# iamwangyabin/hardnetNas

Measured on AMD Instinct MI355X. Metric: Mpatches/s (32×32→128-D) at 1/2/4/8 MI355X; HPatches FPR95 parity, higher is better.
Workload: dtype bf16x3; 1 GPU; Stock HardNet forward, 262144 synthetic 32x32 patches per GPU; model=hardnet, global_batch=262144, per_gpu_batch=262144, parallelism=dp1

## Files before the change

hardnetnas_amd/csrc/hn_hardnet.hip:

```cpp
#include "hn_common.h"
#include "hn_internal.h"

#include <algorithm>
#include <cstdlib>

template <bool NORM>
__global__ __launch_bounds__(256) void k_stem(const float* __restrict__ in, float* __restrict__ out,
                                              const float* __restrict__ w,
                                              const float* __restrict__ b,
                                              float eps) {
  __shared__ float tile[34 * 34];
  __shared__ float red[8];
  const int t = threadIdx.x;
  const size_t p = blockIdx.x;
  const float4 v = reinterpret_cast<const float4*>(in + p * 1024)[t];
  for (int i = t; i < 34 * 34; i += 256) tile[i] = 0.f;
  float mean = 0.f, sd = 1.f;
  if (NORM) {
    float s = wave_sum(v.x + v.y + v.z + v.w);
    if ((t & 63) == 0) red[t >> 6] = s;
    __syncthreads();
    mean = (red[0] + red[1] + red[2] + red[3]) * (1.f / 1024.f);
    const float d0 = v.x - mean, d1 = v.y - mean, d2 = v.z - mean, d3 = v.w - mean;
    float q = wave_sum(d0 * d0 + d1 * d1 + d2 * d2 + d3 * d3);
// ... 756 lines not shown
      w0l[j] = (__bf16)(v - (float)w0h[j]);
    }
#pragma unroll
    for (int i = 0; i < 16; ++i) b16[i] = stem_b[8 * (i >> 2) + 4 * h + (i & 3)];
  }
  auto stem_loads = [&](int s) {
    int p0, y0;
    tile_of(s, p0, y0);
    if (p0 == cur_patch) return;
    const float4* pp = reinterpret_cast<const float4*>(in + (size_t)p0 * 1024) + lane;
    pv[0] = pp[0]; pv[1] = pp[64]; pv[2] = pp[128]; pv[3] = pp[192];
  };
  auto stem_write = [&](int s, char* dst) {
    int p0, y0;
    tile_of(s, p0, y0);
    if (p0 != cur_patch) {
    cur_patch = p0;
    float mean = 0.f, sd = 1.f;
    if (eps >= 0.f) {
      float a = 0.f;
#pragma unroll
      for (int k = 0; k < 4; ++k) a += (pv[k].x + pv[k].y) + (pv[k].z + pv[k].w);
      mean = wave_sum(a) * (1.f / 1024.f);
      float q = 0.f;
#pragma unroll
      for (int k = 0; k < 4; ++k) {
        const float d0 = pv[k].x - mean, d1 = pv[k].y - mean, d2 = pv[k].z - mean,
                    d3 = pv[k].w - mean;
        q += (d0 * d0 + d1 * d1) + (d2 * d2 + d3 * d3);
      }
      sd = sqrtf(wave_sum(q) * (1.f / 1023.f)) + eps;
    }
    const float inv = 1.f / sd;
#define HN_PUT(K)                                                                          \
  {                                                                                        \
    const int q4 = 4 * (lane + 64 * K), y = q4 >> 5, x = q4 & 31;                          \
    float* d = pt + (y + 1) * 34 + x + 1;                                                  \
    d[0] = (pv[K].x - mean) * inv; d[1] = (pv[K].y - mean) * inv;                           \
    d[2] = (pv[K].z - mean) * inv; d[3] = (pv[K].w - mean) * inv;                           \
  }
    HN_PUT(0) HN_PUT(1) HN_PUT(2) HN_PUT(3)
#undef HN_PUT
    }
    constexpr int NPIX = C::RIN * C::NCOLS;
    constexpr int NT0 = (NPIX + 31) / 32;
#pragma unroll 1
    for (int t = pw_; t < NT0; t += C::NWP) {
      const int pix = t * 32 + r;
      const int wr = pix / C::NCOLS, wc = pix % C::NCOLS;
      const int y = y0 - 1 + wr, x = wc - 1;
      const bool inside = pix < NPIX && (unsigned)y < 32u && (unsigned)x < 32u;
      const int yc = inside ? y : 0, xc = inside ? x : 0;
      bf16x8 xh, xl;
#pragma unroll
      for (int j = 0; j < 8; ++j) {
        const int tap = 8 * h + j;
        const float v = tap < 9 ? pt[(yc + tap / 3) * 34 + xc + tap % 3] : 0.f;
        xh[j] = (__bf16)v;
        xl[j] = (__bf16)(v - (float)xh[j]);
      }
      const f32x16 c0 = mfma3(w0h, w0l, xh, xl, f32x16{});
      if (pix < NPIX) {
        char* o = dst + wr * C::RS + wc * 80 + 8 * h;
#pragma unroll
        for (int q = 0; q < 4; ++q) {
          bf16x4 oh, ol;
#pragma unroll
          for (int j = 0; j < 4; ++j) {
            const float v = inside ? fmaxf(c0[4 * q + j] + b16[4 * q + j], 0.f) : 0.f;
            oh[j] = (__bf16)v;
            ol[j] = (__bf16)(v - (float)oh[j]);
          }
          *reinterpret_cast<uint2*>(o + 16 * q) = __builtin_bit_cast(uint2, oh);
          *reinterpret_cast<uint2*>(o + C::PLANE + 16 * q) = __builtin_bit_cast(uint2, ol);
        }
      }
    }
  };

  if (producer) {
    if constexpr (STEM) {
      static_assert(CIN == 32 && HIN == 32 && S == 1 && NP == 1, "stem fusion is conv1-only");
      for (int i = lane; i < 34 * 34; i += 64) pt[i] = 0.f;
      stem_loads(0);
      stem_write(0, buf0);
    } else {
      produce_loads(0, pf);
      produce_write(buf0, pf);
      if (NS > 1) produce_loads(1, pf);
    }
  } else {
    for (int i = tid; i < COUT; i += C::NWC * 64) reinterpret_cast<float*>(smem + C::BIAS_OFF)[i] = bias[i];
  }
  __syncthreads();

  if (producer) {
    if constexpr ((ABL & 32) != 0) {
    } else if constexpr ((ABL & 8) != 0) {
#pragma unroll 1
      for (int s = 0; s < NS; ++s) __syncthreads();
    } else if constexpr (STEM) {
#pragma unroll 1
      for (int s = 0; s < NS; ++s) {
        if (s + 1 < NS) {
          stem_loads(s + 1);
          stem_write(s + 1, (s & 1) ? buf0 : buf1);
        }
        __syncthreads();
      }
    } else if constexpr (!C::DEEP) {
#pragma unroll 1
      for (int s = 0; s < NS; ++s) {
        if (s + 1 < NS) {
          produce_write((s & 1) ? buf0 : buf1, pf);
          if (s + 2 < NS) produce_loads(s + 2, pf);
        }
        __syncthreads();
        if constexpr (PST)
          if (s % C::NCC == C::NCC - 1) pstore(s, (s & 1) ? buf1 : buf0);
      }
    } else {
#pragma unroll 1
      for (int s = 0; s < NS; s += 2) {
        if (s + 2 < NS) produce_loads(s + 2, pf2);
        if (s + 1 < NS) produce_write(buf1, pf);
        __syncthreads();
        if constexpr (PST)
          if (s % C::NCC == C::NCC - 1) pstore(s, buf0);
        if (s + 1 >= NS) break;
        if (s + 3 < NS) produce_loads(s + 3, pf);
        if (s + 2 < NS) produce_write(buf0, pf2);
        __syncthreads();
        if constexpr (PST)
          if ((s + 1) % C::NCC == C::NCC - 1) pstore(s + 1, buf1);
      }
    }
    return;
  }

  const int wm = wave / WN, wn = wave % WN;
  const float* const sbias = reinterpret_cast<const float*>(smem + C::BIAS_OFF);
  int abase[C::MT], ylr[C::MT];
#pragma unroll
  for (int mt = 0; mt < C::MT; ++mt) {
    const int m = (wm * C::MT + mt) * 32 + r;
    const int np = m / (TR * C::WOUT), rem = m % (TR * C::WOUT);
    const int yl = rem / C::WOUT, xo = rem % C::WOUT;
    abase[mt] = np * C::PS + yl * S * C::RS + xo * PX + (PX == 80 ? h * 16 : 0);
    ylr[mt] = yl;
  }
  constexpr unsigned CHUNK_BYTES = 9 * 2 * C::NTOT * 2 * 64 * 16;
  const __amdgpu_buffer_rsrc_t wr_ = make_rsrc(wp, C::NCC * CHUNK_BYTES);
  const unsigned wvoff = (wn * C::NT * 2 * 64 + lane) * 16;
  f32x16 acc[C::MT][C::NT];
#pragma unroll
  for (int mt = 0; mt < C::MT; ++mt)
#pragma unroll
    for (int nt = 0; nt < C::NT; ++nt) acc[mt][nt] = f32x16{};

  constexpr int NKS = 18;
  auto load_b = [&](int cc, int ksx, uint4 (&dst)[C::NT][2]) {
#pragma unroll
    for (int nt = 0; nt < C::NT; ++nt) {
      const unsigned k = cc * CHUNK_BYTES +
                         (((ABL & 1) ? 0 : ksx) * C::NTOT + nt) * 2 * 64 * 16;
      dst[nt][0] = buf_load16(wr_, wvoff, k);
      dst[nt][1] = buf_load16(wr_, wvoff, k + 64 * 16);
    }
  };
  constexpr int WD = 3;
  static_assert(NKS % WD == 0, "the weight ring runs on across stages");
  uint4 bq[WD][C::NT][2];
#pragma unroll
  for (int k = 0; k + 1 < WD; ++k) load_b(0, k, bq[k]);
#pragma unroll 1
  for (int s = 0; s < NS; ++s) {
    const char* cur = (s & 1) ? buf1 : buf0;
    const int cc = s % C::NCC, ccn = (s + 1) % C::NCC;
    uint4 aq[2][C::MT][2];
    auto load_a = [&](int ksx, uint4 (&dst)[C::MT][2]) {
      const int tap = (ABL & 2) ? 0 : ksx >> 1, ks = (ABL & 2) ? 0 : ksx & 1;
      const int toff = (tap / 3) * C::RS + C::colofs(tap % 3) * PX + (PX == 80 ? ks * 32 : 0);
#pragma unroll
      for (int mt = 0; mt < C::MT; ++mt) {
        const int co = PX == 80 ? 0 : 16 * ((2 * ks + h) ^ ((ylr[mt] + (tap / 3) / S) & 3));
        dst[mt][0] = *reinterpret_cast<const uint4*>(cur + abase[mt] + toff + co);
        dst[mt][1] = *reinterpret_cast<const uint4*>(cur + C::PLANE + abase[mt] + toff + co);
      }
    };
    load_a(0, aq[0]);
#pragma unroll
    for (int ksx = 0; ksx < NKS; ++ksx) {
      if (ksx + WD - 1 < NKS)
        load_b(cc, ksx + WD - 1, bq[(ksx + WD - 1) % WD]);
      else
        load_b(ccn, ksx + WD - 1 - NKS, bq[(ksx + WD - 1) % WD]);
      if (ksx + 1 < NKS) load_a(ksx + 1, aq[(ksx + 1) & 1]);
      __builtin_amdgcn_sched_barrier(0);
      if constexpr (PST) {
        if (ksx == 0 && cc == 0 && s > 0) __builtin_amdgcn_s_barrier();
      }
#pragma unroll
      for (int mt = 0; mt < C::MT; ++mt) {
        const bf16x8 xh = as_bf16x8(aq[ksx & 1][mt][0]), xl = as_bf16x8(aq[ksx & 1][mt][1]);
#pragma unroll
        for (int nt = 0; nt < C::NT; ++nt) {
          if constexpr (ABL & 16)
            acc[mt][nt][0] += __builtin_bit_cast(float, aq[ksx & 1][mt][0].x ^ aq[ksx & 1][mt][1].y ^
                                                           bq[ksx % WD][nt][0].z ^ bq[ksx % WD][nt][1].w);
          else
            acc[mt][nt] = mfma3(as_bf16x8(bq[ksx % WD][nt][0]), as_bf16x8(bq[ksx % WD][nt][1]), xh,
                                xl, acc[mt][nt]);
        }
      }
      __builtin_amdgcn_sched_barrier(0);
    }
    if (PST && cc == C::NCC - 1) {
      __syncthreads();
      char* stg = const_cast<char*>(cur);
#pragma unroll
      for (int nt = 0; nt < C::NT; ++nt) {
        float4 bv[4];
#pragma unroll
        for (int q = 0; q < 4; ++q)
          bv[q] = *reinterpret_cast<const float4*>(sbias + (wn * C::NT + nt) * 32 + 8 * q + 4 * h);
#pragma unroll
        for (int mt = 0; mt < C::MT; ++mt) {
          char* o = stage_at(stg, (wm * C::MT + mt) * 32 + r) + ((wn * C::NT + nt) * 32 + 4 * h) * 4;
#pragma unroll
          for (int q = 0; q < 4; ++q) {
            float4 v;
            v.x = fmaxf(acc[mt][nt][4 * q + 0] + bv[q].x, relu_lo);
            v.y = fmaxf(acc[mt][nt][4 * q + 1] + bv[q].y, relu_lo);
            v.z = fmaxf(acc[mt][nt][4 * q + 2] + bv[q].z, relu_lo);
            v.w = fmaxf(acc[mt][nt][4 * q + 3] + bv[q].w, relu_lo);
            *reinterpret_cast<float4*>(o + 32 * q) = v;
          }
          acc[mt][nt] = f32x16{};
        }
      }
      __syncthreads();
      continue;
    }
    if (cc == C::NCC - 1) {
      int p0, y0;
      tile_of(s, p0, y0);
      float* obase = out + ((size_t)(p0 * C::HOUT + y0) * C::WOUT + wm * C::MT * 32 + r) * COUT +
                     wn * C::NT * 32 + 4 * h;
#pragma unroll
      for (int nt = 0; nt < C::NT; ++nt) {
        float4 bv[4];
#pragma unroll
        for (int q = 0; q < 4; ++q)
          bv[q] = *reinterpret_cast<const float4*>(sbias + (wn * C::NT + nt) * 32 + 8 * q + 4 * h);
#pragma unroll
        for (int mt = 0; mt < C::MT; ++mt) {
          const bool ok = NP == 1 || p0 + ((wm * C::MT + mt) * 32) / (TR * C::WOUT) < P;
          if (ok) {
#pragma unroll
            for (int q = 0; q < 4; ++q) {
              float4 v;
              v.x = fmaxf(acc[mt][nt][4 * q + 0] + bv[q].x, relu_lo);
              v.y = fmaxf(acc[mt][nt][4 * q + 1] + bv[q].y, relu_lo);
              v.z = fmaxf(acc[mt][nt][4 * q + 2] + bv[q].z, relu_lo);
              v.w = fmaxf(acc[mt][nt][4 * q + 3] + bv[q].w, relu_lo);
              if constexpr (CST) {
                float* scr = reinterpret_cast<float*>(smem + 2 * C::BUF) + wave * (C::SCR / 4);
                *reinterpret_cast<float4*>(scr + r * C::SROW + 8 * q + 4 * h) = v;
              } else if (!(ABL & 4) || v.x == 1234.5f) {
                *reinterpret_cast<float4*>(obase + (size_t)mt * 32 * COUT + nt * 32 + 8 * q) = v;
              }
            }
          }
          if (CST && ok) {
            __builtin_amdgcn_wave_barrier();
            asm volatile("" ::: "memory");
            const float* scr = reinterpret_cast<const float*>(smem + 2 * C::BUF) + wave * (C::SCR / 4);
            float* ob = out + ((size_t)(p0 * C::HOUT + y0) * C::WOUT + (wm * C::MT + mt) * 32) * COUT +
                        (wn * C::NT + nt) * 32;
#pragma unroll
            for (int k = 0; k < 4; ++k) {
              const int pl = 8 * k + (lane >> 3), c4 = lane & 7;
              *reinterpret_cast<float4*>(ob + (size_t)pl * COUT + 4 * c4) =
                  *reinterpret_cast<const float4*>(scr + pl * C::SROW + 4 * c4);
            }
            __builtin_amdgcn_wave_barrier();
            asm volatile("" ::: "memory");
          }
          acc[mt][nt] = f32x16{};
        }
      }
    }
    if constexpr (!(ABL & 32)) __syncthreads();
  }
  if constexpr (PST) __builtin_amdgcn_s_barrier();
}

template <int K>
__global__ __launch_bounds__(256) void k_head(const float* __restrict__ a, float* __restrict__ out,
                                              const uint4* __restrict__ wp,
                                              const float* __restrict__ bias, int P, float l2eps) {
  __shared__ float ssq[2][64];
  const int tid = threadIdx.x, lane = tid & 63, wave = tid >> 6;
  const int wm = wave >> 1, wn = wave & 1;
  const int r = lane & 31, h = lane >> 5;
  const int pbase = blockIdx.x * 64 + wm * 32;
  const int pa = min(pbase + r, P - 1);
  const float* arow = a + (size_t)pa * K + h * 8;
  f32x16 acc[2] = {f32x16{}, f32x16{}};
#pragma unroll 4
  for (int ks = 0; ks < K / 16; ++ks) {
    const float4 x0 = *reinterpret_cast<const float4*>(arow + ks * 16);
    const float4 x1 = *reinterpret_cast<const float4*>(arow + ks * 16 + 4);
    uint4 hi, lo;
    split8(x0, x1, hi, lo);
    const bf16x8 ah = as_bf16x8(hi), al = as_bf16x8(lo);
#pragma unroll
    for (int nt = 0; nt < 2; ++nt) {
      const int idx = ((ks * 4 + wn * 2 + nt) * 2) * 64 + lane;
      acc[nt] = mfma3(ah, al, as_bf16x8(wp[idx]), as_bf16x8(wp[idx + 64]), acc[nt]);
    }
  }
  float b0 = bias[wn * 64 + r], b1 = bias[wn * 64 + 32 + r];
  float part[16];
#pragma unroll
  for (int i = 0; i < 16; ++i) {
    acc[0][i] += b0;
    acc[1][i] += b1;
    part[i] = half_sum(acc[0][i] * acc[0][i] + acc[1][i] * acc[1][i]);
  }
  if (r == 0) {
#pragma unroll
    for (int i = 0; i < 16; ++i) ssq[wn][wm * 32 + (i & 3) + 8 * (i >> 2) + 4 * h] = part[i];
  }
  __syncthreads();
#pragma unroll
  for (int i = 0; i < 16; ++i) {
    const int row = (i & 3) + 8 * (i >> 2) + 4 * h;
    const int p = pbase + row;
    const float norm = sqrtf(ssq[0][wm * 32 + row] + ssq[1][wm * 32 + row] + l2eps);
    if (p < P) {
      out[(size_t)p * 128 + wn * 64 + r] = acc[0][i] / norm;
      out[(size_t)p * 128 + wn * 64 + 32 + r] = acc[1][i] / norm;
    }
  }
}

template <int K, bool F16>
__global__ __launch_bounds__(256) void k_head2(const float* __restrict__ a, float* __restrict__ out,
                                               const uint4* __restrict__ wp,
                                               const float* __restrict__ bias, int P, float l2eps) {
  constexpr int KC = 32, NCH = K / KC;
  constexpr int AROW = 80;
  constexpr int APLANE = 64 * AROW;
  constexpr int ABYTES = 2 * APLANE;
  constexpr int BBYTES = 2 * 4 * 2 * 64 * 16;
  constexpr int BUF = ABYTES + BBYTES;
  __shared__ __attribute__((aligned(16))) char smem[2 * BUF];
  __shared__ float ssq[2][64];
  const int tid = threadIdx.x, lane = tid & 63, wave = tid >> 6;
  const int wm = wave >> 1, wn = wave & 1;
  const int r = lane & 31, h = lane >> 5;
  const int pbase = blockIdx.x * 64;
  const int arow0 = tid >> 3, acol = (tid & 7) * 4;
  const int pa0 = min(pbase + arow0, P - 1), pa1 = min(pbase + arow0 + 32, P - 1);
  float4 ra0, ra1;
  uint4 rb0, rb1, rb2, rb3;
#define HN_LOAD_CHUNK(c)                                                                   \
  {                                                                                        \
    ra0 = *reinterpret_cast<const float4*>(a + (size_t)pa0 * K + (c) * KC + acol);         \
    ra1 = *reinterpret_cast<const float4*>(a + (size_t)pa1 * K + (c) * KC + acol);         \
    const uint4* wc_ = wp + (size_t)(c) * 1024 + tid;                                      \
    rb0 = wc_[0]; rb1 = wc_[256]; rb2 = wc_[512]; rb3 = wc_[768];                          \
  }
  auto put_row = [&](char* buf, int row, const float4 v) {
    uint2 hv, lv;
    if (F16) {
      typedef _Float16 f16x4 __attribute__((ext_vector_type(4)));
      f16x4 hi, lo;
      hi[0] = (_Float16)v.x; lo[0] = (_Float16)(v.x - (float)hi[0]);
      hi[1] = (_Float16)v.y; lo[1] = (_Float16)(v.y - (float)hi[1]);
      hi[2] = (_Float16)v.z; lo[2] = (_Float16)(v.z - (float)hi[2]);
      hi[3] = (_Float16)v.w; lo[3] = (_Float16)(v.w - (float)hi[3]);
      hv = __builtin_bit_cast(uint2, hi);
      lv = __builtin_bit_cast(uint2, lo);
    } else {
      bf16x4 hi, lo;
      hi[0] = (__bf16)v.x; lo[0] = (__bf16)(v.x - (float)hi[0]);
      hi[1] = (__bf16)v.y; lo[1] = (__bf16)(v.y - (float)hi[1]);
      hi[2] = (__bf16)v.z; lo[2] = (__bf16)(v.z - (float)hi[2]);
      hi[3] = (__bf16)v.w; lo[3] = (__bf16)(v.w - (float)hi[3]);
      hv = __builtin_bit_cast(uint2, hi);
      lv = __builtin_bit_cast(uint2, lo);
    }
    *reinterpret_cast<uint2*>(buf + row * AROW + acol * 2) = hv;
    *reinterpret_cast<uint2*>(buf + APLANE + row * AROW + acol * 2) = lv;
  };
#define HN_STORE_CHUNK(buf)                                                                \
  {                                                                                        \
    put_row(buf, arow0, ra0);                                                              \
    put_row(buf, arow0 + 32, ra1);                                                         \
    uint4* bd_ = reinterpret_cast<uint4*>(buf + ABYTES) + tid;                             \
    bd_[0] = rb0; bd_[256] = rb1; bd_[512] = rb2; bd_[768] = rb3;                          \
  }
  f32x16 acc[2] = {f32x16{}, f32x16{}};
  HN_LOAD_CHUNK(0)
  HN_STORE_CHUNK(smem)
  __syncthreads();
#pragma unroll 1
  for (int c = 0; c < NCH; ++c) {
    const char* cur = smem + (c & 1) * BUF;
    if (c + 1 < NCH) HN_LOAD_CHUNK(c + 1)
#pragma unroll
    for (int ks = 0; ks < 2; ++ks) {
      const int aoff = (wm * 32 + r) * AROW + ks * 32 + h * 16;
      const uint4 ah = *reinterpret_cast<const uint4*>(cur + aoff);
      const uint4 al = *reinterpret_cast<const uint4*>(cur + APLANE + aoff);
#pragma unroll
      for (int nt = 0; nt < 2; ++nt) {
        const int boff = ABYTES + (((ks * 4 + wn * 2 + nt) * 2) * 64 + lane) * 16;
        const uint4 bh = *reinterpret_cast<const uint4*>(cur + boff);
        const uint4 bl = *reinterpret_cast<const uint4*>(cur + boff + 64 * 16);
        if (F16)
          acc[nt] = mfma3_f16(as_f16x8(ah), as_f16x8(al), as_f16x8(bh), as_f16x8(bl), acc[nt]);
        else
          acc[nt] = mfma3(as_bf16x8(ah), as_bf16x8(al), as_bf16x8(bh), as_bf16x8(bl), acc[nt]);
      }
    }
    if (c + 1 < NCH) HN_STORE_CHUNK(smem + ((c + 1) & 1) * BUF)
    __syncthreads();
  }
#undef HN_LOAD_CHUNK
#undef HN_STORE_CHUNK
  const float b0 = bias[wn * 64 + r], b1 = bias[wn * 64 + 32 + r];
  float part[16];
#pragma unroll
  for (int i = 0; i < 16; ++i) {
    acc[0][i] += b0;
    acc[1][i] += b1;
    part[i] = half_sum(acc[0][i] * acc[0][i] + acc[1][i] * acc[1][i]);
  }
  if (r == 0) {
#pragma unroll
    for (int i = 0; i < 16; ++i) ssq[wn][wm * 32 + (i & 3) + 8 * (i >> 2) + 4 * h] = part[i];
  }
  __syncthreads();
// ... 612 lines not shown
```

hardnetnas_amd/csrc/hn_wino1.hip:

```cpp
#include "hn_common.h"
#include "hn_internal.h"

namespace {

template <int CIN, int COUT, int H, int NP, int WM, int WN, bool CST>
struct W1Cfg {
  static constexpr int TR = H;
  static constexpr int NTX = H / 2;
  static constexpr int BM = NP * TR * NTX;
  static constexpr int MT = BM / WM / 32, NT = COUT / WN / 32;
  static constexpr int NTOT = COUT / 32, NCC = CIN / 32;
  static constexpr int XROW = NTX * 64;
  static constexpr int RS = 4 * XROW;
  static constexpr int PS = TR * RS;
  static constexpr int ZROW = NP * PS;
  static constexpr int PLANE = ZROW + RS;
  static constexpr int BUF = 2 * PLANE;
  static constexpr int NWC = WM * WN, NWP = 4, NTHR = (NWC + NWP) * 64, PTHR = NWP * 64;
  static constexpr int UNITS = NP * TR * NTX * 4;
  static_assert(64 % (4 * NTX) == 0 && PTHR % (4 * NTX) == 0, "a row's units share one wave");
  static constexpr int UPT = (UNITS + PTHR - 1) / PTHR;
  static constexpr bool DEEP = UPT <= 2;
  static constexpr int SROW = 36;
  static constexpr int SCR_OFF = 2 * BUF;
  static constexpr int SCR = CST ? 32 * SROW * 4 : 0;
  static constexpr int BIAS_OFF = SCR_OFF + NWC * SCR;
  static constexpr int SMEM = BIAS_OFF + COUT * 4;
  static constexpr int NKS = 24;
  static constexpr unsigned CHUNK_BYTES = NKS * NTOT * 2 * 64 * 16;
  static_assert(SMEM <= 160 * 1024, "LDS");
  static_assert(MT >= 1 && NT >= 1 && MT * WM * 32 == BM && NT * WN * 32 == COUT, "tiling");
  static_assert((TR * NTX) % 32 == 0 && 32 % NTX == 0, "an M tile = 32 / NTX whole rows of one patch");
  static_assert(RS % 256 == 0, "image rows on 256-byte boundaries (the bank-conflict argument)");
};

template <int CIN, int COUT, int H, int NP, int WM, int WN, bool CST, int WD = 3, int ABL = 0>
__global__ __launch_bounds__((WM * WN + 4) * 64) void k_conv_w1(const float* __restrict__ in, float* __restrict__ out,
                                                                const uint4* __restrict__ wp,
                                                                const float* __restrict__ bias, int P) {
  using C = W1Cfg<CIN, COUT, H, NP, WM, WN, CST>;
  constexpr int TR = C::TR;
  extern __shared__ __attribute__((aligned(16))) char smem[];
  const int tid = threadIdx.x, lane = tid & 63;
  const int wave = __builtin_amdgcn_readfirstlane(tid >> 6);
  const bool producer = wave >= C::NWC;
  const int r = lane & 31, h = lane >> 5;
  const int nwg = gridDim.x, rb = xcd_remap(blockIdx.x, nwg);
  const int ntiles = (P + NP - 1) / NP;
  const int my_tiles = rb < ntiles ? (ntiles - 1 - rb) / nwg + 1 : 0;
  const int NS = my_tiles * C::NCC;
  if (NS == 0) return;
  char* const buf0 = smem;
  char* const buf1 = smem + C::BUF;
  auto tile_of = [&](int s) { return (rb + (s / C::NCC) * nwg) * NP; };

  const int ptid = tid - C::NWC * 64;
  float4 pf[C::UPT][6], pf2[C::UPT][6];
  constexpr unsigned PATCH_BYTES = (unsigned)H * H * CIN * 4, OOB = 0x80000000u;
  auto produce_loads = [&](int s, float4 (&d)[C::UPT][6]) {
    const bool live = s < NS;
    const int p0 = live ? tile_of(s) : 0;
    const int cc = s % C::NCC;
    const int nval = !live ? 0 : P - p0 < NP ? P - p0 : NP;
    const __amdgpu_buffer_rsrc_t rs = make_rsrc(in + (size_t)p0 * H * H * CIN, (unsigned)nval * PATCH_BYTES);
#pragma unroll
    for (int k = 0; k < C::UPT; ++k) {
      const int u = ptid + k * C::PTHR;
      const int g = u & 3, t = (u >> 2) % C::NTX, rest = (u >> 2) / C::NTX;
      const int y = rest % TR, np = rest / TR;
      const bool rowok = C::UNITS % C::PTHR == 0 || u < C::UNITS;
#pragma unroll
      for (int j = 0; j < 3; ++j) {
        const int x = 2 * t - 1 + j;
        const bool ok = rowok && (j < 2 || t == C::NTX - 1) && (unsigned)x < (unsigned)H;
        const unsigned vo = ok ? (unsigned)(((np * H + y) * H + x) * CIN + cc * 32 + g * 8) * 4u : OOB;
        d[k][2 * j] = __builtin_bit_cast(float4, buf_load16(rs, vo, 0));
        d[k][2 * j + 1] = __builtin_bit_cast(float4, buf_load16(rs, vo, 16));
      }
    }
  };
  auto shfl4 = [&](const float4& v) {
    return make_float4(__shfl_down(v.x, 4, 64), __shfl_down(v.y, 4, 64), __shfl_down(v.z, 4, 64),
                       __shfl_down(v.w, 4, 64));
  };
  auto produce_write = [&](char* dst, const float4 (&d)[C::UPT][6]) {
#pragma unroll
    for (int k = 0; k < C::UPT; ++k) {
      const int u = ptid + k * C::PTHR;
      const int g = u & 3, t = (u >> 2) % C::NTX, rest = (u >> 2) / C::NTX;
      const int y = rest % TR, np = rest / TR;
      const bool last = t == C::NTX - 1;
      const float4 z = make_float4(0.f, 0.f, 0.f, 0.f);
      float4 dd[4][2];
#pragma unroll
      for (int i = 0; i < 2; ++i) {
        const float4 n0 = shfl4(d[k][i]), n1 = shfl4(d[k][2 + i]);
        dd[0][i] = d[k][i];
        dd[1][i] = d[k][2 + i];
        dd[2][i] = last ? d[k][4 + i] : n0;
        dd[3][i] = last ? z : n1;
      }
      if (C::UNITS % C::PTHR == 0 || u < C::UNITS) {
        const int off = np * C::PS + y * C::RS + t * 64 + 16 * (g ^ ((y + 1) & 3));
#pragma unroll
        for (int xi = 0; xi < 4; ++xi) {
          float4 v[2];
#pragma unroll
          for (int i = 0; i < 2; ++i) {
            const float4 d0 = dd[0][i], d1 = dd[1][i], d2 = dd[2][i], d3 = dd[3][i];
            if (xi == 0) v[i] = make_float4(d0.x - d2.x, d0.y - d2.y, d0.z - d2.z, d0.w - d2.w);
            if (xi == 1) v[i] = make_float4(d1.x + d2.x, d1.y + d2.y, d1.z + d2.z, d1.w + d2.w);
            if (xi == 2) v[i] = make_float4(d2.x - d1.x, d2.y - d1.y, d2.z - d1.z, d2.w - d1.w);
            if (xi == 3) v[i] = make_float4(d1.x - d3.x, d1.y - d3.y, d1.z - d3.z, d1.w - d3.w);
          }
          uint4 hi, lo;
          split8(v[0], v[1], hi, lo);
          *reinterpret_cast<uint4*>(dst + off + xi * C::XROW) = hi;
          *reinterpret_cast<uint4*>(dst + C::PLANE + off + xi * C::XROW) = lo;
        }
      }
    }
  };

  for (int i = tid; i < 4 * C::RS / 16; i += C::NTHR) {
    const int q = i / (C::RS / 16), o = (i % (C::RS / 16)) * 16;
    *reinterpret_cast<uint4*>(smem + (q >> 1) * C::BUF + (q & 1) * C::PLANE + C::ZROW + o) = make_uint4(0, 0, 0, 0);
  }
  if constexpr ((ABL & 64) != 0) {
    if (!producer) __builtin_amdgcn_s_setprio(1);
  }
  if constexpr ((ABL & 128) != 0) {
    if (producer) __builtin_amdgcn_s_setprio(1);
  }
  if (producer) {
    if constexpr ((ABL & 1) != 0) {
#pragma unroll 1
      for (int s = 0; s <= NS; ++s) __syncthreads();
      return;
    }
    produce_loads(0, pf);
    produce_write(buf0, pf);
    produce_loads(1, pf);
    __syncthreads();
    if constexpr (!C::DEEP) {
#pragma unroll 1
      for (int s = 0; s < NS; ++s) {
        produce_write((s & 1) ? buf0 : buf1, pf);
        produce_loads(s + 2, pf);
        __syncthreads();
      }
    } else {
#pragma unroll 1
      for (int s = 0; s < NS; s += 2) {
        produce_loads(s + 2, pf2);
        produce_write(buf1, pf);
        __syncthreads();
        if (s + 1 >= NS) break;
        produce_loads(s + 3, pf);
        produce_write(buf0, pf2);
        __syncthreads();
      }
    }
    return;
  }

  for (int i = tid; i < COUT; i += C::NWC * 64) reinterpret_cast<float*>(smem + C::BIAS_OFF)[i] = bias[i];
  __syncthreads();
  if constexpr ((ABL & 16) != 0) {
#pragma unroll 1
    for (int s = 0; s < NS; ++s) __syncthreads();
    return;
  }
  const int wm = wave / WN, wn = wave % WN;
  const float* const sbias = reinterpret_cast<const float*>(smem + C::BIAS_OFF);
  int ylr[C::MT], vo[C::MT][3][2];
#pragma unroll
  for (int mt = 0; mt < C::MT; ++mt) {
    const int m = (wm * C::MT + mt) * 32 + r;
    const int np = m / (TR * C::NTX), rem = m % (TR * C::NTX);
    ylr[mt] = rem / C::NTX;
#pragma unroll
    for (int ky = 0; ky < 3; ++ky) {
      const int wr = ylr[mt] + ky;
      const int rowb = (wr >= 1 && wr <= TR) ? np * C::PS + (wr - 1) * C::RS : C::ZROW;
#pragma unroll
      for (int ks = 0; ks < 2; ++ks) {
        vo[mt][ky][ks] = rowb + (rem % C::NTX) * 64 + 16 * ((2 * ks + h) ^ (wr & 3));
        asm volatile("" : "+v"(vo[mt][ky][ks]));
      }
    }
  }
  const __amdgpu_buffer_rsrc_t wr_ = make_rsrc(wp, C::NCC * C::CHUNK_BYTES);
  const unsigned wvoff = (wn * C::NT * 2 * 64 + lane) * 16;
  f32x16 y0a[C::MT][C::NT], y1a[C::MT][C::NT], ma[C::MT][C::NT];
#pragma unroll
  for (int mt = 0; mt < C::MT; ++mt)
#pragma unroll
    for (int nt = 0; nt < C::NT; ++nt) y0a[mt][nt] = y1a[mt][nt] = ma[mt][nt] = f32x16{};

  auto load_b = [&](int cc, int kx, uint4 (&dst)[C::NT][2]) {
#pragma unroll
    for (int nt = 0; nt < C::NT; ++nt) {
      const unsigned k = cc * C::CHUNK_BYTES + (((ABL & 4) ? 0 : kx) * C::NTOT + nt) * 2 * 64 * 16;
      dst[nt][0] = buf_load16(wr_, wvoff, k);
      dst[nt][1] = buf_load16(wr_, wvoff, k + 64 * 16);
    }
  };
  static_assert(C::NKS % WD == 0, "the weight ring runs on across stages");
  uint4 bq[WD][C::NT][2];
#pragma unroll
  for (int k = 0; k + 1 < WD; ++k) load_b(0, k, bq[k]);
#pragma unroll 1
  for (int s = 0; s < NS; ++s) {
    const char* cur = (s & 1) ? buf1 : buf0;
    const int cc = s % C::NCC, ccn = (s + 1) % C::NCC;
    uint4 aq[2][C::MT][2];
    auto load_a = [&](int kx, uint4 (&dst)[C::MT][2]) {
      const int xi = kx / 6, ky = (kx % 6) >> 1, ks = kx & 1;
#pragma unroll
      for (int mt = 0; mt < C::MT; ++mt) {
        const char* pa = cur + vo[mt][ky][ks];
        dst[mt][0] = *reinterpret_cast<const uint4*>(pa + xi * C::XROW);
        dst[mt][1] = *reinterpret_cast<const uint4*>(pa + (C::PLANE + xi * C::XROW));
      }
    };
    load_a(0, aq[0]);
#pragma unroll
    for (int kx = 0; kx < C::NKS; ++kx) {
      if constexpr ((ABL & 32) != 0) {
      } else if (kx + WD - 1 < C::NKS)
        load_b(cc, kx + WD - 1, bq[(kx + WD - 1) % WD]);
      else
        load_b(ccn, kx + WD - 1 - C::NKS, bq[(kx + WD - 1) % WD]);
      if (kx + 1 < C::NKS) load_a(kx + 1, aq[(kx + 1) & 1]);
      __builtin_amdgcn_sched_barrier(0);
      const int xi = kx / 6;
      if (kx == 12) {
#pragma unroll
        for (int mt = 0; mt < C::MT; ++mt)
#pragma unroll
          for (int nt = 0; nt < C::NT; ++nt) {
            y0a[mt][nt] += ma[mt][nt];
            y1a[mt][nt] += ma[mt][nt];
          }
      }
#pragma unroll
      for (int mt = 0; mt < C::MT; ++mt) {
        const bf16x8 xh = as_bf16x8(aq[kx & 1][mt][0]), xl = as_bf16x8(aq[kx & 1][mt][1]);
#pragma unroll
        for (int nt = 0; nt < C::NT; ++nt) {
          const bf16x8 wh = as_bf16x8(bq[kx % WD][nt][0]), wl = as_bf16x8(bq[kx % WD][nt][1]);
          if constexpr ((ABL & 2) != 0)
            y0a[mt][nt][0] += __builtin_bit_cast(float, aq[kx & 1][mt][0].x ^ aq[kx & 1][mt][1].y ^
                                                            bq[kx % WD][nt][0].z ^ bq[kx % WD][nt][1].w);
          else if (xi == 0)
            y0a[mt][nt] = mfma3(wh, wl, xh, xl, y0a[mt][nt]);
          else if (xi == 3)
            y1a[mt][nt] = mfma3(wh, wl, xh, xl, y1a[mt][nt]);
          else
            ma[mt][nt] = mfma3(wh, wl, xh, xl, (kx % 6 == 0) ? f32x16{} : ma[mt][nt]);
        }
      }
      __builtin_amdgcn_sched_barrier(0);
    }
#pragma unroll
    for (int mt = 0; mt < C::MT; ++mt)
#pragma unroll
      for (int nt = 0; nt < C::NT; ++nt) {
        y0a[mt][nt] += ma[mt][nt];
        y1a[mt][nt] -= ma[mt][nt];
      }
    if (cc == C::NCC - 1) {
      const int p0 = tile_of(s);
#pragma unroll
      for (int nt = 0; nt < C::NT; ++nt) {
        float4 bv[4];
#pragma unroll
        for (int q = 0; q < 4; ++q)
          bv[q] = *reinterpret_cast<const float4*>(sbias + (wn * C::NT + nt) * 32 + 8 * q + 4 * h);
#pragma unroll
        for (int mt = 0; mt < C::MT; ++mt) {
          const int m0 = (wm * C::MT + mt) * 32;
          const int np = m0 / (TR * C::NTX), yb = (m0 % (TR * C::NTX)) / C::NTX;
          if ((NP == 1 || p0 + np < P) && ((ABL & 8) == 0 || y0a[mt][nt][0] == 1234.5f)) {
            float* const ob = out + (((size_t)p0 + np) * H + yb) * H * COUT + (wn * C::NT + nt) * 32;
#pragma unroll
            for (int par = 0; par < 2; ++par) {
              const f32x16& yv = par ? y1a[mt][nt] : y0a[mt][nt];
              float4 v[4];
#pragma unroll
              for (int q = 0; q < 4; ++q)
                v[q] = make_float4(relu0(yv[4 * q + 0] + bv[q].x), relu0(yv[4 * q + 1] + bv[q].y),
                                   relu0(yv[4 * q + 2] + bv[q].z), relu0(yv[4 * q + 3] + bv[q].w));
              if constexpr (CST) {
                float* scr = reinterpret_cast<float*>(smem + C::SCR_OFF) + wave * (C::SCR / 4);
#pragma unroll
                for (int q = 0; q < 4; ++q) *reinterpret_cast<float4*>(scr + r * C::SROW + 8 * q + 4 * h) = v[q];
                __builtin_amdgcn_wave_barrier();
                asm volatile("" ::: "memory");
#pragma unroll
                for (int k = 0; k < 4; ++k) {
                  const int ml = 8 * k + (lane >> 3), c4 = lane & 7;
                  const int px = (ml / C::NTX) * H + 2 * (ml % C::NTX) + par;
                  *reinterpret_cast<float4*>(ob + (size_t)px * COUT + 4 * c4) =
                      *reinterpret_cast<const float4*>(scr + ml * C::SROW + 4 * c4);
                }
                __builtin_amdgcn_wave_barrier();
                asm volatile("" ::: "memory");
              } else {
                const int px = (r / C::NTX) * H + 2 * (r % C::NTX) + par;
#pragma unroll
                for (int q = 0; q < 4; ++q)
                  *reinterpret_cast<float4*>(ob + (size_t)px * COUT + 8 * q + 4 * h) = v[q];
              }
            }
          }
          y0a[mt][nt] = y1a[mt][nt] = f32x16{};
        }
      }
    }
    __syncthreads();
  }
}

template <int L, int CIN, int COUT, int H, int NP, int WM, int WN, bool CST, int WD, int ABL>
hipError_t launch_w1(const HardnetDev& d, const float* in, float* out, int P, float, hipStream_t st) {
  using C = W1Cfg<CIN, COUT, H, NP, WM, WN, CST>;
  if (!d.wino1[L]) return hipErrorInvalidValue;
  return hn_launch_persistent<&k_conv_w1<CIN, COUT, H, NP, WM, WN, CST, WD, ABL>, C::NTHR, C::SMEM>(
      (P + NP - 1) / NP, st, in, out, static_cast<const uint4*>(d.wino1[L]), d.bias[L], P);
}

#ifdef HN_EXPERIMENTS
template <int CIN, int COUT, int H, int NP, int WN>
struct W4Cfg {
  static constexpr int NTX = H / 4;
  static constexpr int POS = NP * H * NTX;
  static constexpr int MT = POS / 16;
  static constexpr int NCC = CIN / 32;
  static constexpr int NT = COUT / 16 / WN;
  static constexpr int RB = NTX * 64;
  static constexpr int HR = H + 2;
  static constexpr int XB = HR * RB;
  static constexpr int PLANE = NP * 6 * XB;
  static constexpr int BUF = 2 * PLANE;
  static constexpr int NWC = WN, NWP = 4, NTHR = (NWC + NWP) * 64, PTHR = NWP * 64;
  static constexpr int UNITS = NP * H * NTX * 4;
  static constexpr int UPT = UNITS / PTHR;
  static constexpr bool DEEP = UPT <= 2;
  static constexpr int SMEM = 2 * BUF;
  static constexpr int NKS = 18;
  static constexpr unsigned KSTEP_BYTES = (COUT / 16) * 2 * 64 * 16;
  static constexpr unsigned CHUNK_BYTES = NKS * KSTEP_BYTES;
  static_assert(RB == 256, "the bank-conflict argument assumes 256-byte image rows");
  static_assert(UNITS % PTHR == 0 && UPT >= 1, "whole units per producer thread");
  static_assert(POS % 16 == 0 && NT >= 1 && NT * WN * 16 == COUT, "tiling");
  static_assert(SMEM <= 160 * 1024, "LDS");
};

__host__ __device__ constexpr int w4_xi(int xo) { return xo == 0 ? 0 : xo == 1 ? 5 : xo - 1; }

template <int CIN, int COUT, int H, int NP, int WN, int WD, int ABL = 0>
__global__ __launch_bounds__((WN + 4) * 64) void k_conv_w4(const float* __restrict__ in, float* __restrict__ out,
                                                           const uint4* __restrict__ wp,
                                                           const float* __restrict__ bias, int P) {
  using C = W4Cfg<CIN, COUT, H, NP, WN>;
  constexpr int NTX = C::NTX;
  extern __shared__ __attribute__((aligned(16))) char smem[];
  const int tid = threadIdx.x, lane = tid & 63;
  const int wave = __builtin_amdgcn_readfirstlane(tid >> 6);
  const bool producer = wave >= C::NWC;
  const int nwg = gridDim.x, rb = xcd_remap(blockIdx.x, nwg);
  const int ntiles = (P + NP - 1) / NP;
  const int my_tiles = rb < ntiles ? (ntiles - 1 - rb) / nwg + 1 : 0;
  const int NS = my_tiles * C::NCC;
  if (NS == 0) return;
  char* const buf0 = smem;
  char* const buf1 = smem + C::BUF;
  auto tile_of = [&](int s) { return (rb + (s / C::NCC) * nwg) * NP; };

  constexpr int ZCH = C::RB / 16, NZ = 2 * 2 * NP * 6 * 2 * ZCH;
  for (int i = tid; i < NZ; i += C::NTHR) {
    const int q = i % ZCH, rest = i / ZCH;
    const int row = (rest & 1) ? C::HR - 1 : 0, blk = (rest >> 1) % (NP * 6), bp = (rest >> 1) / (NP * 6);
    *reinterpret_cast<uint4*>(smem + bp * C::PLANE + blk * C::XB + row * C::RB + q * 16) = make_uint4(0, 0, 0, 0);
  }

  if (producer) {
    if constexpr ((ABL & 1) != 0) {
#pragma unroll 1
      for (int s = 0; s <= NS; ++s) __syncthreads();
      return;
    }
    const int ptid = tid - C::NWC * 64;
    float4 pf[C::UPT][10], pf2[C::UPT][10];
    constexpr unsigned PATCH_BYTES = (unsigned)H * H * CIN * 4, OOB = 0x80000000u;
    auto produce_loads = [&](int s, float4 (&d)[C::UPT][10]) {
      const bool live = s < NS;
      const int p0 = live ? tile_of(s) : 0;
      const int cc = s % C::NCC;
      const int nval = !live ? 0 : P - p0 < NP ? P - p0 : NP;
      const __amdgpu_buffer_rsrc_t rs = make_rsrc(in + (size_t)p0 * H * H * CIN, (unsigned)nval * PATCH_BYTES);
#pragma unroll
      for (int k = 0; k < C::UPT; ++k) {
        const int u = ptid + k * C::PTHR;
        const int g = u & 3, t = (u >> 2) % NTX, rest = (u >> 2) / NTX;
        const int y = rest % H, np = rest / H;
#pragma unroll
        for (int j = 0; j < 5; ++j) {
          const int x = 4 * t - 1 + j;
          const bool ok = (j < 4 || t == NTX - 1) && (unsigned)x < (unsigned)H;
          const unsigned vo = ok ? (unsigned)(((np * H + y) * H + x) * CIN + cc * 32 + g * 8) * 4u : OOB;
          d[k][2 * j] = __builtin_bit_cast(float4, buf_load16(rs, vo, 0));
          d[k][2 * j + 1] = __builtin_bit_cast(float4, buf_load16(rs, vo, 16));
        }
      }
    };
    auto shfl4 = [&](const float4& v) {
      return make_float4(__shfl_down(v.x, 4, 64), __shfl_down(v.y, 4, 64), __shfl_down(v.z, 4, 64),
                         __shfl_down(v.w, 4, 64));
    };
    auto produce_write = [&](char* dst, const float4 (&d)[C::UPT][10]) {
#pragma unroll
      for (int k = 0; k < C::UPT; ++k) {
        const int u = ptid + k * C::PTHR;
        const int g = u & 3, t = (u >> 2) % NTX, rest = (u >> 2) / NTX;
        const int y = rest % H, np = rest / H;
        const bool last = t == NTX - 1;
        float4 dd[6][2];
#pragma unroll
        for (int i = 0; i < 2; ++i) {
          const float4 n0 = shfl4(d[k][i]), n1 = shfl4(d[k][2 + i]);
          dd[0][i] = d[k][i];
          dd[1][i] = d[k][2 + i];
          dd[2][i] = d[k][4 + i];
          dd[3][i] = d[k][6 + i];
          dd[4][i] = last ? d[k][8 + i] : n0;
          dd[5][i] = last ? make_float4(0.f, 0.f, 0.f, 0.f) : n1;
        }
        const int off = np * 6 * C::XB + (y + 1) * C::RB + t * 64 + 16 * (g ^ (2 * (y & 1)));
#pragma unroll
        for (int xi = 0; xi < 6; ++xi) {
          float4 v[2];
#pragma unroll
          for (int i = 0; i < 2; ++i) {
            auto tr = [&](float d0, float d1, float d2, float d3, float d4, float d5) {
              switch (xi) {
                case 0: return fmaf(0.25f, d0, fmaf(-1.25f, d2, d4));
                case 1: return fmaf(-0.25f, d1 + d2, d3 + d4);
                case 2: return fmaf(0.25f, d1 - d2, d4 - d3);
                case 3: return fmaf(-0.5f, d1 - d3, d4 - d2);
                case 4: return fmaf(0.5f, d1 - d3, d4 - d2);
                default: return fmaf(0.25f, d1, fmaf(-1.25f, d3, d5));
              }
            };
            v[i] = make_float4(tr(dd[0][i].x, dd[1][i].x, dd[2][i].x, dd[3][i].x, dd[4][i].x, dd[5][i].x),
                               tr(dd[0][i].y, dd[1][i].y, dd[2][i].y, dd[3][i].y, dd[4][i].y, dd[5][i].y),
                               tr(dd[0][i].z, dd[1][i].z, dd[2][i].z, dd[3][i].z, dd[4][i].z, dd[5][i].z),
                               tr(dd[0][i].w, dd[1][i].w, dd[2][i].w, dd[3][i].w, dd[4][i].w, dd[5][i].w));
          }
          uint4 hi, lo;
          split8(v[0], v[1], hi, lo);
          *reinterpret_cast<uint4*>(dst + off + xi * C::XB) = hi;
          *reinterpret_cast<uint4*>(dst + C::PLANE + off + xi * C::XB) = lo;
        }
      }
    };
    produce_loads(0, pf);
    produce_write(buf0, pf);
    produce_loads(1, pf);
// ... 242 lines not shown
```

Baseline: 5.476 Mpatches/s.

## Restructure conv stage loops per tile and interleave Winograd folds with MFMA

Both persistent conv kernels now loop over tiles and then input-channel chunks, with a compile-time first-chunk stage that zeroes the accumulators through the MFMA C operand. This replaces explicit accumulator clears and the per-stage last-chunk branching. In the Winograd kernel, the 3-MFMA bf16x3 sequence is fully unrolled with static_for, and the y0/y1/m fold additions are split into small VALU groups. sched_group_barrier then interleaves those groups between MFMAs so the fold VALU work hides behind matrix work rather than running as a serial pass after each stage. The change adds template complexity and a static_assert that limits the Winograd kernel to two accumulator tiles per wave.

New measurement: 5.604 Mpatches/s, median of 6. +2.3%, better.

```diff
diff --git a/hardnetnas_amd/csrc/hn_hardnet.hip b/hardnetnas_amd/csrc/hn_hardnet.hip
--- a/hardnetnas_amd/csrc/hn_hardnet.hip
+++ b/hardnetnas_amd/csrc/hn_hardnet.hip
@@ -932,12 +932,6 @@
   constexpr unsigned CHUNK_BYTES = 9 * 2 * C::NTOT * 2 * 64 * 16;
   const __amdgpu_buffer_rsrc_t wr_ = make_rsrc(wp, C::NCC * CHUNK_BYTES);
   const unsigned wvoff = (wn * C::NT * 2 * 64 + lane) * 16;
-  f32x16 acc[C::MT][C::NT];
-#pragma unroll
-  for (int mt = 0; mt < C::MT; ++mt)
-#pragma unroll
-    for (int nt = 0; nt < C::NT; ++nt) acc[mt][nt] = f32x16{};
-
   constexpr int NKS = 18;
   auto load_b = [&](int cc, int ksx, uint4 (&dst)[C::NT][2]) {
 #pragma unroll
@@ -953,10 +947,10 @@
   uint4 bq[WD][C::NT][2];
 #pragma unroll
   for (int k = 0; k + 1 < WD; ++k) load_b(0, k, bq[k]);
-#pragma unroll 1
-  for (int s = 0; s < NS; ++s) {
+  f32x16 acc[C::MT][C::NT];
+  auto stage = [&](auto first, int s, int cc, int ccn) {
+    constexpr bool FIRST = decltype(first)::value;
     const char* cur = (s & 1) ? buf1 : buf0;
-    const int cc = s % C::NCC, ccn = (s + 1) % C::NCC;
     uint4 aq[2][C::MT][2];
     auto load_a = [&](int ksx, uint4 (&dst)[C::MT][2]) {
       const int tap = (ABL & 2) ? 0 : ksx >> 1, ks = (ABL & 2) ? 0 : ksx & 1;
@@ -978,26 +972,38 @@
       if (ksx + 1 < NKS) load_a(ksx + 1, aq[(ksx + 1) & 1]);
       __builtin_amdgcn_sched_barrier(0);
       if constexpr (PST) {
-        if (ksx == 0 && cc == 0 && s > 0) __builtin_amdgcn_s_barrier();
+        if (FIRST && ksx == 0 && s > 0) __builtin_amdgcn_s_barrier();
       }
 #pragma unroll
       for (int mt = 0; mt < C::MT; ++mt) {
         const bf16x8 xh = as_bf16x8(aq[ksx & 1][mt][0]), xl = as_bf16x8(aq[ksx & 1][mt][1]);
 #pragma unroll
         for (int nt = 0; nt < C::NT; ++nt) {
-          if constexpr (ABL & 16)
+          const f32x16 c = FIRST && ksx == 0 ? f32x16{} : acc[mt][nt];
+          if constexpr (ABL & 16) {
+            acc[mt][nt] = c;
             acc[mt][nt][0] += __builtin_bit_cast(float, aq[ksx & 1][mt][0].x ^ aq[ksx & 1][mt][1].y ^
                                                            bq[ksx % WD][nt][0].z ^ bq[ksx % WD][nt][1].w);
-          else
-            acc[mt][nt] = mfma3(as_bf16x8(bq[ksx % WD][nt][0]), as_bf16x8(bq[ksx % WD][nt][1]), xh,
-                                xl, acc[mt][nt]);
+          } else {
+            acc[mt][nt] = mfma3(as_bf16x8(bq[ksx % WD][nt][0]), as_bf16x8(bq[ksx % WD][nt][1]), xh, xl, c);
+          }
         }
       }
       __builtin_amdgcn_sched_barrier(0);
     }
-    if (PST && cc == C::NCC - 1) {
+  };
+#pragma unroll 1
+  for (int t = 0; t < my_tiles; ++t) {
+    const int s0 = t * C::NCC, s = s0 + C::NCC - 1;
+    stage(std::true_type{}, s0, 0, C::NCC > 1 ? 1 : 0);
+#pragma unroll 1
+    for (int cc = 1; cc < C::NCC; ++cc) {
+      if constexpr (!(ABL & 32)) __syncthreads();
+      stage(std::false_type{}, s0 + cc, cc, (cc + 1) % C::NCC);
+    }
+    if constexpr (PST) {
       __syncthreads();
-      char* stg = const_cast<char*>(cur);
+      char* stg = (s & 1) ? buf1 : buf0;
 #pragma unroll
       for (int nt = 0; nt < C::NT; ++nt) {
         float4 bv[4];
@@ -1016,13 +1022,10 @@
             v.w = fmaxf(acc[mt][nt][4 * q + 3] + bv[q].w, relu_lo);
             *reinterpret_cast<float4*>(o + 32 * q) = v;
           }
-          acc[mt][nt] = f32x16{};
         }
       }
       __syncthreads();
-      continue;
-    }
-    if (cc == C::NCC - 1) {
+    } else {
       int p0, y0;
       tile_of(s, p0, y0);
       float* obase = out + ((size_t)(p0 * C::HOUT + y0) * C::WOUT + wm * C::MT * 32 + r) * COUT +
@@ -1067,11 +1070,10 @@
             __builtin_amdgcn_wave_barrier();
             asm volatile("" ::: "memory");
           }
-          acc[mt][nt] = f32x16{};
         }
       }
-    }
-    if constexpr (!(ABL & 32)) __syncthreads();
+      if constexpr (!(ABL & 32)) __syncthreads();
+    }
   }
   if constexpr (PST) __builtin_amdgcn_s_barrier();
 }
diff --git a/hardnetnas_amd/csrc/hn_wino1.hip b/hardnetnas_amd/csrc/hn_wino1.hip
--- a/hardnetnas_amd/csrc/hn_wino1.hip
+++ b/hardnetnas_amd/csrc/hn_wino1.hip
@@ -34,6 +34,24 @@
   static_assert(RS % 256 == 0, "image rows on 256-byte boundaries (the bank-conflict argument)");
 };
 
+template <int... I, class F>
+HN_DEV void static_for_seq(std::integer_sequence<int, I...>, F&& f) {
+  (f(std::integral_constant<int, I>{}), ...);
+}
+template <int N, class F>
+HN_DEV void static_for(F&& f) {
+  static_for_seq(std::make_integer_sequence<int, N>{}, f);
+}
+
+constexpr int w1_lo3(int g) { return g == 0 ? 0 : g == 1 ? 6 : g == 2 ? 11 : 16; }
+constexpr int w1_fold_valu(bool first, int kx, int g) {
+  if (kx == 11 && g >= 3) return 2 * (w1_lo3(g - 2) - w1_lo3(g - 3));
+  if (kx == 12 && g < 3) return 2 * (w1_lo3(g + 1) - w1_lo3(g));
+  if (kx == 18 || kx == 19 || (kx == 0 && !first)) return g < 5 ? 3 : 1;
+  if (kx == 23 && g >= 3) return w1_lo3(g - 2) - w1_lo3(g - 3);
+  return 0;
+}
+
 template <int CIN, int COUT, int H, int NP, int WM, int WN, bool CST, int WD = 3, int ABL = 0>
 __global__ __launch_bounds__((WM * WN + 4) * 64) void k_conv_w1(const float* __restrict__ in, float* __restrict__ out,
                                                                 const uint4* __restrict__ wp,
@@ -192,11 +210,8 @@
   }
   const __amdgpu_buffer_rsrc_t wr_ = make_rsrc(wp, C::NCC * C::CHUNK_BYTES);
   const unsigned wvoff = (wn * C::NT * 2 * 64 + lane) * 16;
-  f32x16 y0a[C::MT][C::NT], y1a[C::MT][C::NT], ma[C::MT][C::NT];
-#pragma unroll
-  for (int mt = 0; mt < C::MT; ++mt)
-#pragma unroll
-    for (int nt = 0; nt < C::NT; ++nt) y0a[mt][nt] = y1a[mt][nt] = ma[mt][nt] = f32x16{};
+  static_assert(C::MT * C::NT == 2, "the fold schedule below is written for two accumulator tiles per wave");
+  f32x16 y0a[2], y1a[2], ma[2];
 
   auto load_b = [&](int cc, int kx, uint4 (&dst)[C::NT][2]) {
 #pragma unroll
@@ -210,10 +225,42 @@
   uint4 bq[WD][C::NT][2];
 #pragma unroll
   for (int k = 0; k + 1 < WD; ++k) load_b(0, k, bq[k]);
-#pragma unroll 1
-  for (int s = 0; s < NS; ++s) {
+
+  auto sadd = [](float a, float b) {
+    float v = a + b;
+    asm("" : "+v"(v));
+    return v;
+  };
+  auto ssub = [](float a, float b) {
+    float v = a - b;
+    asm("" : "+v"(v));
+    return v;
+  };
+  auto fold = [&](auto first_, auto kx_, auto g_) {
+    constexpr bool first = decltype(first_)::value;
+    constexpr int kx = decltype(kx_)::value, g = decltype(g_)::value;
+    if constexpr ((kx == 11 && g >= 3) || (kx == 12 && g < 3)) {
+      constexpr int j = kx == 11 ? 0 : 1, g3 = kx == 11 ? g - 3 : g;
+#pragma unroll
+      for (int i = w1_lo3(g3); i < w1_lo3(g3 + 1); ++i) {
+        y0a[j][i] = sadd(y0a[j][i], ma[j][i]);
+        y1a[j][i] = sadd(first ? 0.f : y1a[j][i], ma[j][i]);
+      }
+    } else if constexpr (kx == 18 || kx == 19) {
+#pragma unroll
+      for (int i = 3 * g; i < 3 * g + 3 && i < 16; ++i) y0a[kx - 18][i] = sadd(y0a[kx - 18][i], ma[kx - 18][i]);
+    } else if constexpr (kx == 23 && g >= 3) {
+#pragma unroll
+      for (int i = w1_lo3(g - 3); i < w1_lo3(g - 2); ++i) y1a[0][i] = ssub(y1a[0][i], ma[0][i]);
+    } else if constexpr (kx == 0 && !first) {
+#pragma unroll
+      for (int i = 3 * g; i < 3 * g + 3 && i < 16; ++i) y1a[1][i] = ssub(y1a[1][i], ma[1][i]);
+    }
+  };
+
+  auto stage = [&](auto first_, int s, int cc, int ccn) {
+    constexpr bool FIRST = decltype(first_)::value;
     const char* cur = (s & 1) ? buf1 : buf0;
-    const int cc = s % C::NCC, ccn = (s + 1) % C::NCC;
     uint4 aq[2][C::MT][2];
     auto load_a = [&](int kx, uint4 (&dst)[C::MT][2]) {
       const int xi = kx / 6, ky = (kx % 6) >> 1, ks = kx & 1;
@@ -225,53 +272,59 @@
       }
     };
     load_a(0, aq[0]);
-#pragma unroll
-    for (int kx = 0; kx < C::NKS; ++kx) {
+    static_for<C::NKS>([&](auto kx_) {
+      constexpr int kx = decltype(kx_)::value, xi = kx / 6;
       if constexpr ((ABL & 32) != 0) {
-      } else if (kx + WD - 1 < C::NKS)
+      } else if constexpr (kx + WD - 1 < C::NKS)
         load_b(cc, kx + WD - 1, bq[(kx + WD - 1) % WD]);
       else
         load_b(ccn, kx + WD - 1 - C::NKS, bq[(kx + WD - 1) % WD]);
-      if (kx + 1 < C::NKS) load_a(kx + 1, aq[(kx + 1) & 1]);
+      if constexpr (kx + 1 < C::NKS) load_a(kx + 1, aq[(kx + 1) & 1]);
       __builtin_amdgcn_sched_barrier(0);
-      const int xi = kx / 6;
-      if (kx == 12) {
-#pragma unroll
-        for (int mt = 0; mt < C::MT; ++mt)
-#pragma unroll
-          for (int nt = 0; nt < C::NT; ++nt) {
-            y0a[mt][nt] += ma[mt][nt];
-            y1a[mt][nt] += ma[mt][nt];
+      static_for<6>([&](auto g_) {
+        constexpr int g = decltype(g_)::value, j = g / 3, p = g % 3, mt = j / C::NT, nt = j % C::NT;
+        const bf16x8 x = as_bf16x8(aq[kx & 1][mt][p == 1 ? 1 : 0]), w = as_bf16x8(bq[kx % WD][nt][p == 0 ? 1 : 0]);
+        f32x16& acc = xi == 0 ? y0a[j] : xi == 3 ? y1a[j] : ma[j];
+        constexpr bool zero = p == 0 && (kx == 6 || kx == 12 || (kx == 0 && FIRST));
+        if constexpr ((ABL & 2) != 0) {
+          if (FIRST && kx == 0 && p == 0) y0a[j] = y1a[j] = ma[j] = f32x16{};
+          if (p == 0)
+            y0a[j][0] += __builtin_bit_cast(float, aq[kx & 1][mt][0].x ^ aq[kx & 1][mt][1].y ^
+                                                       bq[kx % WD][nt][0].z ^ bq[kx % WD][nt][1].w);
+        } else {
+          acc = __builtin_amdgcn_mfma_f32_32x32x16_bf16(w, x, zero ? f32x16{} : acc, 0, 0, 0);
+          constexpr int nv = w1_fold_valu(FIRST, kx, g);
+          if constexpr (nv > 0) {
+            fold(first_, kx_, g_);
+            __builtin_amdgcn_sched_group_barrier(0x008, 1, 0);
+            __builtin_amdgcn_sched_group_barrier(0x002, nv, 0);
+          } else if constexpr (w1_fold_valu(FIRST, kx, 0) + w1_fold_valu(FIRST, kx, 5) > 0) {
+            __builtin_amdgcn_sched_group_barrier(0x008, 1, 0);
           }
-      }
-#pragma unroll
-      for (int mt = 0; mt < C::MT; ++mt) {
-        const bf16x8 xh = as_bf16x8(aq[kx & 1][mt][0]), xl = as_bf16x8(aq[kx & 1][mt][1]);
-#pragma unroll
-        for (int nt = 0; nt < C::NT; ++nt) {
-          const bf16x8 wh = as_bf16x8(bq[kx % WD][nt][0]), wl = as_bf16x8(bq[kx % WD][nt][1]);
-          if constexpr ((ABL & 2) != 0)
-            y0a[mt][nt][0] += __builtin_bit_cast(float, aq[kx & 1][mt][0].x ^ aq[kx & 1][mt][1].y ^
-                                                            bq[kx % WD][nt][0].z ^ bq[kx % WD][nt][1].w);
-          else if (xi == 0)
-            y0a[mt][nt] = mfma3(wh, wl, xh, xl, y0a[mt][nt]);
-          else if (xi == 3)
-            y1a[mt][nt] = mfma3(wh, wl, xh, xl, y1a[mt][nt]);
-          else
-            ma[mt][nt] = mfma3(wh, wl, xh, xl, (kx % 6 == 0) ? f32x16{} : ma[mt][nt]);
-        }
-      }
+        }
+      });
       __builtin_amdgcn_sched_barrier(0);
-    }
-#pragma unroll
-    for (int mt = 0; mt < C::MT; ++mt)
-#pragma unroll
-      for (int nt = 0; nt < C::NT; ++nt) {
-        y0a[mt][nt] += ma[mt][nt];
-        y1a[mt][nt] -= ma[mt][nt];
-      }
-    if (cc == C::NCC - 1) {
+    });
+  };
+  auto fold_last = [&] {
+#pragma unroll
+    for (int i = 0; i < 16; ++i) y1a[1][i] = ssub(y1a[1][i], ma[1][i]);
+  };
+#pragma unroll 1
+  for (int t = 0; t < my_tiles; ++t) {
+    const int s0 = t * C::NCC, s = s0 + C::NCC - 1;
+    stage(std::true_type{}, s0, 0, C::NCC > 1 ? 1 : 0);
+#pragma unroll 1
+    for (int cc = 1; cc < C::NCC; ++cc) {
+      __syncthreads();
+      stage(std::false_type{}, s0 + cc, cc, (cc + 1) % C::NCC);
+    }
+    if constexpr ((ABL & 2) == 0) fold_last();
+    {
       const int p0 = tile_of(s);
+      int le = lane;
+      asm volatile("" : "+v"(le));
+      const int r = le & 31, h = le >> 5;
 #pragma unroll
       for (int nt = 0; nt < C::NT; ++nt) {
         float4 bv[4];
@@ -282,11 +335,11 @@
         for (int mt = 0; mt < C::MT; ++mt) {
           const int m0 = (wm * C::MT + mt) * 32;
           const int np = m0 / (TR * C::NTX), yb = (m0 % (TR * C::NTX)) / C::NTX;
-          if ((NP == 1 || p0 + np < P) && ((ABL & 8) == 0 || y0a[mt][nt][0] == 1234.5f)) {
+          if ((NP == 1 || p0 + np < P) && ((ABL & 8) == 0 || y0a[mt * C::NT + nt][0] == 1234.5f)) {
             float* const ob = out + (((size_t)p0 + np) * H + yb) * H * COUT + (wn * C::NT + nt) * 32;
 #pragma unroll
             for (int par = 0; par < 2; ++par) {
-              const f32x16& yv = par ? y1a[mt][nt] : y0a[mt][nt];
+              const f32x16& yv = par ? y1a[mt * C::NT + nt] : y0a[mt * C::NT + nt];
               float4 v[4];
 #pragma unroll
               for (int q = 0; q < 4; ++q)
@@ -300,7 +353,7 @@
                 asm volatile("" ::: "memory");
 #pragma unroll
                 for (int k = 0; k < 4; ++k) {
-                  const int ml = 8 * k + (lane >> 3), c4 = lane & 7;
+                  const int ml = 8 * k + (le >> 3), c4 = le & 7;
                   const int px = (ml / C::NTX) * H + 2 * (ml % C::NTX) + par;
                   *reinterpret_cast<float4*>(ob + (size_t)px * COUT + 4 * c4) =
                       *reinterpret_cast<const float4*>(scr + ml * C::SROW + 4 * c4);
@@ -315,7 +368,6 @@
               }
             }
           }
-          y0a[mt][nt] = y1a[mt][nt] = f32x16{};
         }
       }
     }
```
